# jetuk/pycllp

Hardware: AMD Instinct MI355X
Metric: LPs solved/sec (higher is better)
Workload: dtype f64

## Files before the change

### pycllp_amd/csrc/ipm_group.inc

```

#ifndef PYCLLP_SPLITJ
#define PYCLLP_SPLITJ 6
#endif
#ifndef PYCLLP_GRAM_UNROLL
#define PYCLLP_GRAM_UNROLL 4
#endif
#ifndef PYCLLP_AT_RB
#define PYCLLP_AT_RB 4
#endif
#ifndef PYCLLP_A_CB
#define PYCLLP_A_CB 8
#endif
#ifndef PYCLLP_SOLVE_PRIO
#define PYCLLP_SOLVE_PRIO 2
#endif
#ifndef PYCLLP_FACTOR_PRIO
#define PYCLLP_FACTOR_PRIO 2
#endif
#ifndef PYCLLP_FACTOR_PRIO_HSD
#define PYCLLP_FACTOR_PRIO_HSD 3
#endif
#ifndef PYCLLP_WPB
#define PYCLLP_WPB 8
#endif

template <int MP, int NP, bool SL = false>
struct GeoG {
    static_assert(MP == 16 || MP == 32, "row padding must be 16 or 32");
    static_assert(NP % MP == 0 && NP % 8 == 0 && NP <= 128, "column padding must be a multiple of MP and 8, <= 128");
    static_assert(!SL || NP >= 2 * MP, "the slack-aware variant needs at least one dense register");
    static constexpr int G = 64 / MP;
    static constexpr int NCG = NP / MP;
    static constexpr int ND = SL ? NP - MP : NP;
    static constexpr int NCD = ND / MP;
    static constexpr int JB = MP / 16;
    static constexpr int KS = ND / 4;
    static constexpr int AS = ND + 1;
    static constexpr int AIMG = MP * AS;
    static constexpr bool SWZ = (MP == 32);
    static constexpr int MS = SWZ ? MP : MP + 2;
    __host__ __device__ static constexpr int sidx(int row, int col) {
        return SWZ ? row * MS + (col ^ ((row & 15) << 1)) : row * MS + col;
    }
    static constexpr int SLAB = MP * MS;
    static constexpr int STAGE = 3 * ND;
    static constexpr int STAGE_A = (G * ND > STAGE) ? G * ND : STAGE;
    static constexpr int STAGE_SZ = (2 * G * MP > STAGE_A) ? 2 * G * MP : STAGE_A;
    static constexpr int SHARED = AIMG + ND;
    static constexpr int WSZ = G * SLAB + STAGE_SZ;
    static constexpr size_t lds_bytes(int wpb) { return sizeof(double) * (size_t)(SHARED + wpb * WSZ); }
    __host__ __device__ static constexpr int kpos(int j) { return (j & 3) * KS + (j >> 2); }
};

template <int MP>
__device__ __forceinline__ double grp_sum(double v) {
    asm volatile("" : "+v"(v));
    v += dpp_d<0xB1>(v);
    v += dpp_d<0x4E>(v);
    v += dpp_d<0x141>(v);
    v += dpp_d<0x140>(v);
    if (MP == 32) v += swz_xor16_d(v);
    return v;
}
template <int MP>
__device__ __forceinline__ double grp_max(double v) {
    v = fmax(v, dpp_d<0xB1>(v));
    v = fmax(v, dpp_d<0x4E>(v));
    v = fmax(v, dpp_d<0x141>(v));
    v = fmax(v, dpp_d<0x140>(v));
    if (MP == 32) v = fmax(v, swz_xor16_d(v));
    return v;
}
template <int MP>
__device__ __forceinline__ double grp_bcast(double v, int k, int grp) {
    if (MP == 32) {
        const double a = readlane_d(v, k), b = readlane_d(v, 32 + k);
        return grp ? b : a;
    } else {
        const double a = readlane_d(v, k), b = readlane_d(v, 16 + k), c = readlane_d(v, 32 + k), d = readlane_d(v, 48 + k);
        return (grp & 2) ? ((grp & 1) ? d : c) : ((grp & 1) ? b : a);
    }
}

template <int MP, int NP, bool SL = false>
struct GWave {
    using G_ = GeoG<MP, NP, SL>;
    static constexpr int G = G_::G, NCG = G_::NCG, NCD = G_::NCD, ND = G_::ND, JB = G_::JB, KS = G_::KS, AS = G_::AS, MS = G_::MS;

    const double* Aimg;
    static constexpr bool COLB = MP == 32 && NP <= 96;
    static constexpr bool ROWB = COLB && SL;
    unsigned rb[ROWB ? 16 : 1];
    unsigned xb[COLB ? 16 : 1];
    double* slab;
    double* slab0;
    double* stage;
    int lane, gl, grp, m, n;

    __device__ __forceinline__ int ogl() const { int g = gl; asm volatile("" : "+v"(g)); return g; }

    __device__ __forceinline__ void load_own_row(double (&out)[MP]) const {
        typedef double double2_t __attribute__((ext_vector_type(2)));
        if constexpr (ROWB) {
#pragma unroll
            for (int p2 = 0; p2 < MP / 2; p2++) {
                const double2_t t = *(const __attribute__((address_space(3))) double2_t*)(size_t)rb[p2];
                out[2 * p2] = t[0]; out[2 * p2 + 1] = t[1];
            }
            return;
        }
        const int g = ogl();
        const double2_t* rp = (const double2_t*)(slab + g * MS);
        const int g15 = G_::SWZ ? (g & 15) : 0;
#pragma unroll
        for (int p2 = 0; p2 < MP / 2; p2++) {
            const double2_t t = rp[p2 ^ g15];
            out[2 * p2] = t[0]; out[2 * p2 + 1] = t[1];
        }
    }

    __device__ __forceinline__ void At_times(double u, double (&out)[NCG]) const {
        const int g = ogl();
        stage[grp * MP + g] = u;
        wave_lds_sync();
        unsigned uba = lds_addr(stage + grp * MP);
        asm volatile("" : "+v"(uba));
        const __attribute__((address_space(3))) double* ub = (const __attribute__((address_space(3))) double*)(size_t)uba;
        const double* ac = Aimg + g;
        constexpr int RB = PYCLLP_AT_RB, NB = MP / RB;
        double a0[RB][NCD], a1[RB][NCD], u0[RB], u1[RB];
#define AT_LOAD(A_, U_, I0)                                                                     \
    _Pragma("unroll") for (int ii = 0; ii < RB; ii++) {                                         \
        U_[ii] = ub[(I0) + ii + tok];                                                           \
        _Pragma("unroll") for (int q = 0; q < NCD; q++) A_[ii][q] = ac[((I0) + ii) * AS + MP * q + tok]; \
    }
#define AT_USE(A_, U_)                                                                          \
    _Pragma("unroll") for (int ii = 0; ii < RB; ii++) {                                         \
        asm volatile("" : "+v"(U_[ii]));                                                        \
        _Pragma("unroll") for (int q = 0; q < NCD; q++) asm volatile("" : "+v"(A_[ii][q]));     \
    }                                                                                           \
    asm volatile("" : "+v"(tok));                                                               \
    _Pragma("unroll") for (int ii = 0; ii < RB; ii++)                                           \
        _Pragma("unroll") for (int q = 0; q < NCD; q++) out[q] = fma(A_[ii][q], U_[ii], out[q]); \
    _Pragma("unroll") for (int q = 0; q < NCD; q++) asm volatile("" : "+v"(out[q]));
#pragma unroll
        for (int q = 0; q < NCG; q++) out[q] = 0.0;
        if (SL) out[NCG - 1] = u;
        int tok = 0;
        asm volatile("" : "+v"(tok));
        AT_LOAD(a0, u0, 0)
        static_for<0, NB / 2>([&](auto bc) {
            constexpr int b2 = 2 * decltype(bc)::value;
            AT_LOAD(a1, u1, (b2 + 1) * RB)
            AT_USE(a0, u0)
            if constexpr (b2 + 2 < NB) { AT_LOAD(a0, u0, (b2 + 2) * RB) }
            AT_USE(a1, u1)
        });
#undef AT_LOAD
#undef AT_USE
        wave_lds_sync();
    }

    __device__ __forceinline__ double A_times(const double (&vq)[NCG]) const {
        const int g = ogl();
#pragma unroll
        for (int q = 0; q < NCD; q++) stage[grp * ND + g + MP * q] = vq[q];
        wave_lds_sync();
        unsigned vba = lds_addr(stage + grp * ND);
        asm volatile("" : "+v"(vba));
        const __attribute__((address_space(3))) double* vb = (const __attribute__((address_space(3))) double*)(size_t)vba;
        const double* row = Aimg + g * AS;
        constexpr int CB = (ND % PYCLLP_A_CB == 0) ? PYCLLP_A_CB : 8, NB = ND / CB;
        double a0[CB], a1[CB], v0[CB], v1[CB];
        double acc[4] = {0.0, 0.0, 0.0, 0.0};
#define A_LOAD(A_, V_, J0) \
    _Pragma("unroll") for (int jj = 0; jj < CB; jj++) { A_[jj] = row[(J0) + jj + tok]; V_[jj] = vb[(J0) + jj + tok]; }
#define A_USE(A_, V_)                                                                                          \
    _Pragma("unroll") for (int jj = 0; jj < CB; jj++) { asm volatile("" : "+v"(A_[jj])); asm volatile("" : "+v"(V_[jj])); } \
    asm volatile("" : "+v"(tok));                                                                              \
    _Pragma("unroll") for (int jj = 0; jj < CB; jj++) acc[jj & 3] = fma(A_[jj], V_[jj], acc[jj & 3]);
        int tok = 0;
        asm volatile("" : "+v"(tok));
        A_LOAD(a0, v0, 0)
        static_for<0, (NB + 1) / 2>([&](auto bc) {
            constexpr int b2 = 2 * decltype(bc)::value;
            if constexpr (b2 + 1 < NB) { A_LOAD(a1, v1, (b2 + 1) * CB) }
            A_USE(a0, v0)
            if constexpr (b2 + 2 < NB) { A_LOAD(a0, v0, (b2 + 2) * CB) }
            if constexpr (b2 + 1 < NB) { A_USE(a1, v1) }
        });
#undef A_LOAD
#undef A_USE
        wave_lds_sync();
        return (acc[0] + acc[1]) + (acc[2] + acc[3]) + (SL ? vq[NCG - 1] : 0.0);
    }

    template <bool AX = true>
    __device__ __forceinline__ void gram_one(int g, double (&axp)[JB], double (&adp)[JB]) const {
        int lo0_ = lane;
        asm volatile("" : "+v"(lo0_));
        const int kg = lo0_ >> 4, cc = lo0_ & 15;
        double4_t acc[JB][JB];
#pragma unroll
        for (int I = 0; I < JB; I++) {
            axp[I] = 0.0; adp[I] = 0.0;
#pragma unroll
            for (int J = 0; J < JB; J++) acc[I][J] = (double4_t){0.0, 0.0, 0.0, 0.0};
        }
        const double* px = stage + kg * KS;
        const double* pd = stage + ND + kg * KS;
        const double* pt = stage + 2 * ND + kg * KS;
        const double* arow = Aimg + cc * AS + kg;
        constexpr int SC = (KS % 4 == 0) ? 4 : 2;
#pragma unroll PYCLLP_GRAM_UNROLL
        for (int s0 = 0; s0 < KS; s0 += SC) {
#pragma unroll
            for (int ss = 0; ss < SC; ss++) {
                const int s = s0 + ss;
                const double xk = AX ? px[s] : 0.0, dk = pd[s], tk = pt[s];
                double a[JB], ad[JB];
#pragma unroll
                for (int J = 0; J < JB; J++) {
                    a[J] = arow[16 * J * AS + 4 * s];
                    if (AX) axp[J] = fma(a[J], xk, axp[J]);
                    adp[J] = fma(a[J], tk, adp[J]);
                    ad[J] = a[J] * dk;
                }
#pragma unroll
                for (int I = 0; I < JB; I++)
#pragma unroll
                    for (int J = 0; J <= I; J++)
                        acc[I][J] = __builtin_amdgcn_mfma_f64_16x16x4f64(ad[I], a[J], acc[I][J], 0, 0, 0);
            }
        }
        double* sg = slab0 + g * G_::SLAB;
        int lo_ = lane;
        asm volatile("" : "+v"(lo_));
        const int kg2 = lo_ >> 4, cc2 = lo_ & 15;
        if constexpr (G_::SWZ) {
            const int c0 = cc2 ^ (kg2 << 1);
            double* e0 = sg + kg2 * G_::MS + c0;
            double* e1 = sg + kg2 * G_::MS + (c0 ^ 8);
#pragma unroll
            for (int I = 0; I < JB; I++)
#pragma unroll
                for (int J = 0; J <= I; J++)
#pragma unroll
                    for (int r4 = 0; r4 < 4; r4++)
                        ((r4 & 1) ? e1 : e0)[(16 * I + 4 * r4) * G_::MS + 16 * (J ^ (r4 >> 1))] = acc[I][J][r4];
        } else {
#pragma unroll
            for (int I = 0; I < JB; I++)
#pragma unroll
                for (int J = 0; J <= I; J++)
#pragma unroll
                    for (int r4 = 0; r4 < 4; r4++) {
                        const int row = 16 * I + kg2 + 4 * r4, col = 16 * J + cc2;
                        sg[G_::sidx(row, col)] = acc[I][J][r4];
                    }
        }
#pragma unroll
        for (int J = 0; J < JB; J++) {
            if (AX) {
                axp[J] += __shfl_xor(axp[J], 16, WAVE);
                axp[J] += __shfl_xor(axp[J], 32, WAVE);
            }
            adp[J] += __shfl_xor(adp[J], 16, WAVE);
            adp[J] += __shfl_xor(adp[J], 32, WAVE);
        }
    }

    __device__ __forceinline__ static double top_row_of(double u) {
        const int lo = __double2loint(u), hi = __double2hiint(u);
        auto a = __builtin_amdgcn_permlane16_swap(lo, lo, false, false);
        auto b = __builtin_amdgcn_permlane16_swap(hi, hi, false, false);
        return __hiloint2double(b[0], a[0]);
    }

    template <bool RELF = false>
    __device__ __forceinline__ bool factor_dpp(double (&W)[MP], double beta2, double floor_, bool live, double& rdiag,
                                               const double* fl = nullptr) const {
        rdiag = 1.0;
        constexpr int PRIO_ = RELF ? PYCLLP_FACTOR_PRIO_HSD : PYCLLP_FACTOR_PRIO;
        if constexpr (PRIO_ != 0) __builtin_amdgcn_s_setprio(PRIO_);
        const int go = ogl();
        (void)go;
        double ymax = 0.0;
        static_for<0, MP>([&](auto jc) {
            constexpr int j = decltype(jc)::value;
            const double u = W[j];
            double src = u;
            if constexpr (MP == 32 && j < 16) src = top_row_of(u);
            const double piv = bcast64<j % 16>(src);
            const double aD = RELF ? max_abs<false>(piv, fl[j]) : max_abs<true>(piv, floor_);
            const double rD = fast_rcp(aD);
            constexpr unsigned below32 = (j + 1 < 32) ? (0xFFFFFFFFu << ((j + 1) & 31)) : 0u;
            constexpr unsigned below16 = (j + 1 < 16) ? (((0xFFFFu << ((j + 1) & 15)) & 0xFFFFu) * 0x10001u) : 0u;
            constexpr unsigned MB_ = (MP == 32) ? below32 : below16;
            constexpr unsigned ONE_ = (MP == 32) ? (1u << (j % 32)) : ((1u << (j % 16)) * 0x10001u);
            double l = 0.0;
            asm volatile("" : "+v"(l));
            if constexpr (MP == 16) {
                chain_step_exec<j, MB_, MB_, 1, ONE_, ONE_>(W, 0.0, rD, l, ymax, rdiag);
            } else if constexpr (j < 16) {
                chain_step_exec<j, MB_, MB_, 0, ONE_, ONE_>(*reinterpret_cast<double (*)[16]>(&W[0]), src, rD, l, ymax, rdiag);
                chain_all_neg(*reinterpret_cast<double (*)[16]>(&W[16]), W[j], l);
            } else {
                chain_step_exec<j - 16, MB_, MB_, 1, ONE_, ONE_>(*reinterpret_cast<double (*)[16]>(&W[16]), 0.0, rD, l, ymax, rdiag);
            }
            W[j] = l;
        });
        const bool viol = live && (ymax > beta2);
        if constexpr (PRIO_ != 0) __builtin_amdgcn_s_setprio(0);
        if constexpr (COLB) {
#pragma unroll
            for (int j = 0; j < MP; j++) *(__attribute__((address_space(3))) double*)(size_t)(xb[j & 15] + 256u * (unsigned)(j & ~15)) = W[j];
        } else {
            const int g = ogl();
#pragma unroll
            for (int j = 0; j < MP; j++) slab[G_::sidx(j, g)] = W[j];
        }
        wave_lds_sync();
        return __any(viol);
    }

    __device__ __forceinline__ double factor_guarded_inplace(bool rowok, double beta2, double floor_,
                                                             const double* fl = nullptr) const {
        if (!rowok) slab[G_::sidx(gl, gl)] = 1.0;
        wave_lds_sync();
        double rdiag = 1.0;
#pragma unroll 1
        for (int j = 0; j < MP; j++) {
            const bool below = gl > j;
            const double u = below ? slab[G_::sidx(gl, j)] : 0.0;
            const double piv = slab[G_::sidx(j, j)];
            const double theta = grp_max<MP>(fabs(u));
            const double aD = fmax(fmax(fabs(piv), fl ? fl[j] : floor_), theta * theta / beta2);
            const double rD = fast_rcp(aD);
            const double li = u * rD;
            if (gl == j) rdiag = rD;
#pragma unroll 1
            for (int k = j + 1; k < MP; k++) {
                const double uk = slab[G_::sidx(k, j)];
                if (gl >= k) slab[G_::sidx(gl, k)] = fma(-li, uk, slab[G_::sidx(gl, k)]);
            }
            wave_lds_sync();
            slab[G_::sidx(j, gl)] = below ? li : 0.0;
            wave_lds_sync();
        }
#pragma unroll 1
        for (int k = 0; k < MP; k++) if (k <= gl) slab[G_::sidx(gl, k)] = 0.0;
        wave_lds_sync();
        return rdiag;
    }

    __device__ __forceinline__ double fwd_back(double s, double rdiag) const {
        if constexpr (PYCLLP_SOLVE_PRIO != 0) __builtin_amdgcn_s_setprio(PYCLLP_SOLVE_PRIO);
        double lf[MP];
        if constexpr (COLB) {
#pragma unroll
            for (int k = 0; k < MP - 1; k++) lf[k] = *(const __attribute__((address_space(3))) double*)(size_t)(xb[k & 15] + 256u * (unsigned)(k & ~15));
        } else {
            const int g = ogl();
#pragma unroll
            for (int k = 0; k < MP - 1; k++) lf[k] = slab[G_::sidx(k, g)];
        }
#pragma unroll
        for (int k = 0; k < MP - 1; k++) asm volatile("" : "+v"(lf[k]));
        if constexpr (MP == 16) {
            subst15_up(s, lf);
        } else {
            const bool top = gl < 16;
            if (top) subst15_up(s, lf);
            const double so = swz_xor16_d(s);
            if (!top) {
                s -= dot16_bcast(so, lf);
                subst15_up(s, lf + 16);
            }
        }
        s *= rdiag;
        double lb[MP];
        load_own_row(lb);
#pragma unroll
        for (int i = 1; i < MP; i++) asm volatile("" : "+v"(lb[i]));
        if constexpr (MP == 16) {
            subst15_down(s, lb);
            return s;
        } else {
            const bool top = gl < 16;
            if (!top) subst15_down(s, lb + 16);
            const double so = swz_xor16_d(s);
            if (top) {
                s -= dot16_bcast(so, lb + 16);
                subst15_down(s, lb);
            }
            if constexpr (PYCLLP_SOLVE_PRIO != 0) __builtin_amdgcn_s_setprio(0);
            return s;
        }
    }
};

template <int MP, int NP, bool SL, bool PC = false>
__global__ void __launch_bounds__(PYCLLP_WPB * 64)
ipm_group_kernel(int m, int n, long B, const double* __restrict__ Ag, const double* __restrict__ bg,
                 const double* __restrict__ cg, double* __restrict__ xg, double* __restrict__ yg,
                 double* __restrict__ zg, double* __restrict__ pobj, double* __restrict__ dobj,
                 int* __restrict__ status, int* __restrict__ iters, int* __restrict__ queue, DevOpts o) {
    using G_ = GeoG<MP, NP, SL>;
    constexpr int G = G_::G, NCG = G_::NCG, NCD = G_::NCD, ND = G_::ND, JB = G_::JB, AS = G_::AS;
    const int nd = SL ? n - m : n;
    extern __shared__ __attribute__((aligned(16))) double lds[];
    const int tid = threadIdx.x;
    const int wpb = blockDim.x / WAVE;
    double* Aimg = lds;
    double* colsum = lds + G_::AIMG;
    for (int i = tid; i < G_::AIMG; i += blockDim.x) {
        const int r = i / AS, cidx = i % AS;
        Aimg[i] = (r < m && cidx < nd) ? Ag[(size_t)r * n + cidx] : 0.0;
    }
    __syncthreads();
    for (int j = tid; j < ND; j += blockDim.x) {
        double sacc = 0.0;
        for (int i = 0; i < MP; i++) sacc += Aimg[i * AS + j];
        colsum[j] = sacc;
    }
    __syncthreads();

    GWave<MP, NP, SL> w;
    const int wave = tid / WAVE;
    const int lane = tid & 63, gl = lane & (MP - 1), grp = lane / MP;
    w.lane = lane; w.gl = gl; w.grp = grp; w.m = m; w.n = n;
    w.Aimg = Aimg;
    w.slab0 = lds + G_::SHARED + wave * G_::WSZ;
    w.slab = w.slab0 + grp * G_::SLAB;
    w.stage = w.slab0 + G * G_::SLAB;
    if constexpr (GWave<MP, NP, SL>::COLB) {
#pragma unroll
        for (int cidx = 0; cidx < 16; cidx++) w.xb[cidx] = lds_addr(w.slab) + 8u * (unsigned)G_::sidx(cidx, gl);
    }
    if constexpr (GWave<MP, NP, SL>::ROWB) {
#pragma unroll
        for (int p2 = 0; p2 < 16; p2++) w.rb[p2] = lds_addr(w.slab + gl * G_::MS) + 16u * (unsigned)(p2 ^ (gl & 15));
    }
    for (int i = lane; i < G * G_::SLAB; i += WAVE) w.slab0[i] = 0.0;
    wave_lds_sync();
    const bool rowok = gl < m;
    const bool warm = (o.flags & PYCLLP_FLAG_WARM_START) != 0;
    const bool autoscale = (o.flags & PYCLLP_FLAG_AUTOSCALE) != 0;
    const unsigned long long gmask = (MP == 32) ? 0xFFFFFFFFull : 0xFFFFull;
    STAMP_DECL

    const long nslots = (long)gridDim.x * wpb * G;
    long lp = (long)grp * ((long)gridDim.x * wpb) + (long)blockIdx.x * wpb + wave;
    bool live = lp < B, fresh = live;

    double x[NCG], z[NCG], c[NCG], v[NCG];
    bool ok[NCG];
#pragma unroll
    for (int q = 0; q < NCG; q++) {
        ok[q] = (q < NCD) ? (gl + MP * q < nd) : (gl < m);
        x[q] = 1.0; z[q] = 1.0; c[q] = 0.0; v[q] = 0.0;
    }
    auto gcol = [&](int q, int g_) { return (q < NCD) ? g_ + MP * q : nd + g_; };
    double b = 0.0, y = 0.0;
    double tol_r = 0.0, tol_s = 0.0, etol = 0.0, normr0 = 1e300, norms0 = 1e300;
    double rho_pred = 0.0;
    bool have_pred = false;
    int it = 0;

    while (__any(live)) {
        if (__any(fresh)) {
            if (fresh) {
                const int go = w.ogl();
#pragma unroll
                for (int q = 0; q < NCG; q++) {
                    const int j = gcol(q, go);
                    c[q] = ok[q] ? cg[lp * n + j] : 0.0;
                    x[q] = (warm && ok[q]) ? xg[lp * n + j] : 1.0;
                    z[q] = (warm && ok[q]) ? zg[lp * n + j] : 1.0;
                    v[q] = (q < NCD) ? colsum[go + MP * q] : (rowok ? 1.0 : 0.0);
                }
                b = rowok ? bg[lp * m + go] : 0.0;
                y = rowok ? ((warm && yg) ? yg[lp * m + go] : 1.0) : 0.0;
            }
            if (autoscale) {
                double cm = 0.0;
#pragma unroll
                for (int q = 0; q < NCG; q++) cm = fmax(cm, fabs(c[q]));
                double sb = grp_max<MP>(fabs(b)), sc = grp_max<MP>(cm);
                sb = (sb > 0.0) ? sb : 1.0; sc = (sc > 0.0) ? sc : 1.0;
                if (fresh) {
                    b = b / sb;
#pragma unroll
                    for (int q = 0; q < NCG; q++) c[q] = c[q] / sc;
                    if (warm) {
                        y = y / sc;
#pragma unroll
                        for (int q = 0; q < NCG; q++) { x[q] = x[q] / sb; z[q] = z[q] / sc; }
                    }
                }
            }
            double c2 = 0.0;
#pragma unroll
            for (int q = 0; q < NCG; q++) c2 = fma(c[q], c[q], c2);
            const double nb2 = grp_sum<MP>(b * b), nc2 = grp_sum<MP>(c2);
            double vw[NCG];
            if (warm) w.At_times(y, vw);
            if (fresh) {
                tol_r = o.eps * (1.0 + sqrt(nb2));
                tol_s = o.eps * (1.0 + sqrt(nc2));
                etol = o.refine_tol * (1.0 + sqrt(nb2));
                normr0 = 1e300; norms0 = 1e300; it = 0; have_pred = false;
                if (warm) {
#pragma unroll
                    for (int q = 0; q < NCG; q++) v[q] = vw[q];
                }
            }
            fresh = false;
            STAMP(9)
        }

        double s2 = 0.0, gam = 0.0, pp = 0.0;
#pragma unroll
        for (int q = 0; q < NCG; q++) {
            const double sg = ok[q] ? c[q] - v[q] + z[q] : 0.0;
            s2 = fma(sg, sg, s2);
            gam += ok[q] ? x[q] * z[q] : 0.0;
            pp += c[q] * (ok[q] ? x[q] : 0.0);
        }
        s2 = grp_sum<MP>(s2); gam = grp_sum<MP>(gam);
        const double po = grp_sum<MP>(pp);
        const double du = grp_sum<MP>(b * y);
        const double norms = sqrt(s2);
        double mu = PC ? 0.0 : o.delta * gam / (double)(n + m);

        auto finalize = [&](int stat_) {
            double sb = 1.0, sc = 1.0;
            const int go = w.ogl();
            int gro = grp;
            asm volatile("" : "+v"(gro));
            if (autoscale) {
                double cm = 0.0;
#pragma unroll
                for (int q = 0; q < NCG; q++) cm = fmax(cm, ok[q] ? fabs(cg[lp * n + gcol(q, go)]) : 0.0);
                sb = grp_max<MP>(rowok ? fabs(bg[lp * m + go]) : 0.0);
                sc = grp_max<MP>(cm);
                sb = (sb > 0.0) ? sb : 1.0; sc = (sc > 0.0) ? sc : 1.0;
            }
#pragma unroll
            for (int q = 0; q < NCG; q++) {
                const int j = gcol(q, go);
                if (ok[q]) {
                    xg[lp * n + j] = x[q] * sb;
                    if (zg) zg[lp * n + j] = z[q] * sc;
                }
            }
            if (yg && rowok) yg[lp * m + go] = y * sc;
            if (go == 0) {
                if (pobj) pobj[lp] = po * (sb * sc);
                if (dobj) dobj[lp] = du * (sb * sc);
                status[lp] = stat_;
                if (iters) iters[lp] = it;
            }
            int nxt = 0;
            if (go == 0) nxt = atomicAdd(queue, 1);
            nxt = __shfl(nxt, gro * MP, WAVE);
            lp = nslots + (long)nxt;
            live = lp < B;
            fresh = live;
            have_pred = false;
            if (!live) {
#pragma unroll
// ... 215 lines not shown
```

### pycllp_amd/csrc/ipm_group_bounded.inc

```

#ifndef PYCLLP_WPB_BOUNDED
#define PYCLLP_WPB_BOUNDED 4
#endif

template <int MP, int NP>
__global__ void __launch_bounds__(PYCLLP_WPB_BOUNDED * 64)
ipm_bounded_kernel(int m, int n, long B, const double* __restrict__ Ag, const double* __restrict__ bg,
                   const double* __restrict__ cg, const double* __restrict__ ug, double* __restrict__ xg,
                   double* __restrict__ yg, double* __restrict__ zg, double* __restrict__ sg, double* __restrict__ pobj,
                   double* __restrict__ dobj, int* __restrict__ status, int* __restrict__ iters, int* __restrict__ queue,
                   DevOpts o) {
    using G_ = GeoG<MP, NP, true>;
    constexpr int G = G_::G, NCG = G_::NCG, NCD = G_::NCD, ND = G_::ND, JB = G_::JB, AS = G_::AS;
    const int nd = n - m;
    extern __shared__ __attribute__((aligned(16))) double lds[];
    const int tid = threadIdx.x;
    const int wpb = blockDim.x / WAVE;
    double* Aimg = lds;
    double* colsum = lds + G_::AIMG;
    for (int i = tid; i < G_::AIMG; i += blockDim.x) {
        const int r = i / AS, cidx = i % AS;
        Aimg[i] = (r < m && cidx < nd) ? Ag[(size_t)r * n + cidx] : 0.0;
    }
    __syncthreads();
    for (int j = tid; j < ND; j += blockDim.x) {
        double sacc = 0.0;
        for (int i = 0; i < MP; i++) sacc += Aimg[i * AS + j];
        colsum[j] = sacc;
    }
    __syncthreads();

    GWave<MP, NP, true> w;
    const int wave = tid / WAVE;
    const int lane = tid & 63, gl = lane & (MP - 1), grp = lane / MP;
    w.lane = lane; w.gl = gl; w.grp = grp; w.m = m; w.n = n;
    w.Aimg = Aimg;
    w.slab0 = lds + G_::SHARED + wave * G_::WSZ;
    w.slab = w.slab0 + grp * G_::SLAB;
    w.stage = w.slab0 + G * G_::SLAB;
    if constexpr (GWave<MP, NP, true>::COLB) {
#pragma unroll
        for (int cidx = 0; cidx < 16; cidx++) w.xb[cidx] = lds_addr(w.slab) + 8u * (unsigned)G_::sidx(cidx, gl);
    }
    if constexpr (GWave<MP, NP, true>::ROWB) {
#pragma unroll
        for (int p2 = 0; p2 < 16; p2++) w.rb[p2] = lds_addr(w.slab + gl * G_::MS) + 16u * (unsigned)(p2 ^ (gl & 15));
    }
    for (int i = lane; i < G * G_::SLAB; i += WAVE) w.slab0[i] = 0.0;
    wave_lds_sync();
    const bool rowok = gl < m;
    const bool autoscale = (o.flags & PYCLLP_FLAG_AUTOSCALE) != 0;
    const unsigned long long gmask = (MP == 32) ? 0xFFFFFFFFull : 0xFFFFull;

    const long nslots = (long)gridDim.x * wpb * G;
    long lp = (long)grp * ((long)gridDim.x * wpb) + (long)blockIdx.x * wpb + wave;
    bool live = lp < B, fresh = live;

    double x[NCG], z[NCG], t[NCG], s[NCG], u[NCG], c[NCG], v[NCG];
    bool ok[NCG];
#pragma unroll
    for (int q = 0; q < NCG; q++) {
        ok[q] = (q < NCD) ? (gl + MP * q < nd) : (gl < m);
        x[q] = 1.0; z[q] = 1.0; t[q] = 1.0; s[q] = 1.0; u[q] = 0.0; c[q] = 0.0; v[q] = 0.0;
    }
    auto act = [&](int q) { return u[q] > 0.0; };
    auto bnd = [&](int q) { return u[q] > 0.0 && u[q] < HUGE_VAL; };
    auto gcol = [&](int q, int g_) { return (q < NCD) ? g_ + MP * q : nd + g_; };
    double b = 0.0, y = 0.0;
    double tol_r = 0.0, tol_s = 0.0, tol_u = 0.0, etol = 0.0, normr0 = 1e300, norms0 = 1e300, ncomp = 1.0;
    int it = 0;

    while (__any(live)) {
        if (__any(fresh)) {
            if (fresh) {
                const int go = w.ogl();
#pragma unroll
                for (int q = 0; q < NCG; q++) {
                    const int j = gcol(q, go);
                    c[q] = ok[q] ? cg[lp * n + j] : 0.0;
                    u[q] = ok[q] ? ug[lp * n + j] : 0.0;
                    v[q] = (q < NCD) ? colsum[go + MP * q] : (rowok ? 1.0 : 0.0);
                }
                b = rowok ? bg[lp * m + go] : 0.0;
                y = rowok ? 1.0 : 0.0;
            }
            if (autoscale) {
                double cm = 0.0;
#pragma unroll
                for (int q = 0; q < NCG; q++) cm = fmax(cm, act(q) ? fabs(c[q]) : 0.0);
                double sb = grp_max<MP>(fabs(b)), sc = grp_max<MP>(cm);
                sb = (sb > 0.0) ? sb : 1.0; sc = (sc > 0.0) ? sc : 1.0;
                if (fresh) {
                    b = b / sb;
#pragma unroll
                    for (int q = 0; q < NCG; q++) { c[q] = c[q] / sc; u[q] = u[q] / sb; }
                }
            }
            double c2 = 0.0, u2 = 0.0, nb = 0.0;
#pragma unroll
            for (int q = 0; q < NCG; q++) {
                c2 += act(q) ? c[q] * c[q] : 0.0;
                u2 += bnd(q) ? u[q] * u[q] : 0.0;
                nb += bnd(q) ? 1.0 : 0.0;
            }
            const double nb2 = grp_sum<MP>(b * b), nc2 = grp_sum<MP>(c2), nu2 = grp_sum<MP>(u2), nbs = grp_sum<MP>(nb);
            if (fresh) {
#pragma unroll
                for (int q = 0; q < NCG; q++) {
                    x[q] = bnd(q) ? fmin(1.0, 0.5 * u[q]) : 1.0;
                    t[q] = bnd(q) ? u[q] - x[q] : 1.0;
                    z[q] = 1.0; s[q] = 1.0;
                }
                tol_r = o.eps * (1.0 + sqrt(nb2));
                tol_s = o.eps * (1.0 + sqrt(nc2));
                tol_u = o.eps * (1.0 + sqrt(nu2));
                etol = o.refine_tol * (1.0 + sqrt(nb2));
                ncomp = (double)(n + m) + nbs;
                normr0 = 1e300; norms0 = 1e300; it = 0;
            }
            fresh = false;
        }

        double s2 = 0.0, gam = 0.0, pp = 0.0, tau2 = 0.0, du = b * y;
#pragma unroll
        for (int q = 0; q < NCG; q++) {
            const bool a = act(q), bq = bnd(q);
            const double sgq = a ? c[q] - v[q] + z[q] - (bq ? s[q] : 0.0) : 0.0;
            const double tau = bq ? (u[q] - x[q]) - t[q] : 0.0;
            s2 = fma(sgq, sgq, s2);
            tau2 = fma(tau, tau, tau2);
            gam += a ? x[q] * z[q] : 0.0;
            gam += bq ? s[q] * t[q] : 0.0;
            pp += a ? c[q] * x[q] : 0.0;
            du += bq ? u[q] * s[q] : 0.0;
        }
        s2 = grp_sum<MP>(s2); gam = grp_sum<MP>(gam); tau2 = grp_sum<MP>(tau2);
        const double po = grp_sum<MP>(pp);
        du = grp_sum<MP>(du);
        const double norms = sqrt(s2), ntau = sqrt(tau2);
        const double mu = o.delta * gam / ncomp;

        auto finalize = [&](int stat_) {
            double sb = 1.0, sc = 1.0;
            const int go = w.ogl();
            int gro = grp;
            asm volatile("" : "+v"(gro));
            if (autoscale) {
                double cm = 0.0;
#pragma unroll
                for (int q = 0; q < NCG; q++) cm = fmax(cm, act(q) ? fabs(cg[lp * n + gcol(q, go)]) : 0.0);
                sb = grp_max<MP>(rowok ? fabs(bg[lp * m + go]) : 0.0);
                sc = grp_max<MP>(cm);
                sb = (sb > 0.0) ? sb : 1.0; sc = (sc > 0.0) ? sc : 1.0;
            }
#pragma unroll
            for (int q = 0; q < NCG; q++) {
                const int j = gcol(q, go);
                if (ok[q]) {
                    const bool a = act(q), bq = bnd(q);
                    const double r = c[q] - v[q];
                    xg[lp * n + j] = a ? x[q] * sb : 0.0;
                    if (zg) zg[lp * n + j] = (a ? z[q] : fmax(-r, 0.0)) * sc;
                    if (sg) sg[lp * n + j] = (bq ? s[q] : (a ? 0.0 : fmax(r, 0.0))) * sc;
                }
            }
            if (yg && rowok) yg[lp * m + go] = y * sc;
            if (go == 0) {
                if (pobj) pobj[lp] = po * (sb * sc);
                if (dobj) dobj[lp] = du * (sb * sc);
                status[lp] = stat_;
                if (iters) iters[lp] = it;
            }
            int nxt = 0;
            if (go == 0) nxt = atomicAdd(queue, 1);
            nxt = __shfl(nxt, gro * MP, WAVE);
            lp = nslots + (long)nxt;
            live = lp < B;
            fresh = live;
            if (!live) {
#pragma unroll
                for (int q = 0; q < NCG; q++) { x[q] = 1.0; z[q] = 1.0; t[q] = 1.0; s[q] = 1.0; u[q] = 0.0; c[q] = 0.0; v[q] = 0.0; }
                b = 0.0; y = 0.0;
            }
        };

        double rxk[NCG], rzk[NCG], rtk[NCG];
#pragma unroll
        for (int q = 0; q < NCG; q++) { rxk[q] = fast_rcp(x[q]); rzk[q] = fast_rcp(z[q]); rtk[q] = fast_rcp(t[q]); }
        auto newton_dt = [&](int q, double& dq, double& tq) {
            const bool a = act(q), bq = bnd(q);
            const double tau = (u[q] - x[q]) - t[q];
            if (bq) {
                dq = fast_rcp(fma(z[q], rxk[q], s[q] * rtk[q]));
                tq = c[q] - v[q] + mu * rxk[q] - mu * rtk[q] + (s[q] * rtk[q]) * tau;
            } else {
                dq = x[q] * rzk[q];
                tq = c[q] - v[q] + mu * rxk[q];
            }
            dq = a ? dq : 0.0;
            tq = a ? tq : 0.0;
        };
        auto do_gram = [&](double& Ax_, double& Adt_) {
            double d[NCG], tt[NCG];
#pragma unroll
            for (int q = 0; q < NCG; q++) newton_dt(q, d[q], tt[q]);
#pragma unroll 1
            for (int g = 0; g < G; g++) {
                if (__shfl((int)live, g * MP, WAVE) == 0) continue;
                if (grp == g) {
#pragma unroll
                    for (int q = 0; q < NCD; q++) {
                        const int p = G_::kpos(gl + MP * q);
                        w.stage[p] = act(q) ? x[q] : 0.0;
                        w.stage[ND + p] = d[q];
                        w.stage[2 * ND + p] = d[q] * tt[q];
                    }
                }
                wave_lds_sync();
                double axp[JB], adp[JB];
                w.template gram_one<true>(g, axp, adp);
                wave_lds_sync();
                if (grp == g) {
                    Ax_ = (JB == 1) ? axp[0] : ((gl >> 4) ? axp[JB - 1] : axp[0]);
                    Adt_ = (JB == 1) ? adp[0] : ((gl >> 4) ? adp[JB - 1] : adp[0]);
                }
            }
            Ax_ += act(NCG - 1) ? x[NCG - 1] : 0.0;
            Adt_ += d[NCG - 1] * tt[NCG - 1];
            w.slab[G_::sidx(gl, gl)] += d[NCG - 1];
            wave_lds_sync();
        };
        double Ax = 0.0, Adt = 0.0;
        do_gram(Ax, Adt);
        const double rho = b - Ax;
        const double normr = sqrt(grp_sum<MP>(rho * rho));

        int stat = PYCLLP_STATUS_ITERATION_LIMIT;
        bool fin = true;
        if (!(isfinite(normr) && isfinite(norms) && isfinite(gam) && isfinite(ntau))) stat = PYCLLP_STATUS_NUMERICAL;
        else if (normr <= tol_r && norms <= tol_s && gam <= o.eps * (1.0 + fabs(po)) && ntau <= tol_u) stat = PYCLLP_STATUS_OPTIMAL;
        else if (normr > 10.0 * normr0 && normr > PYCLLP_GROWTH_FLOOR * tol_r) stat = PYCLLP_STATUS_PRIMAL_INFEASIBLE;
        else if (norms > 10.0 * norms0 && norms > PYCLLP_GROWTH_FLOOR * tol_s) stat = PYCLLP_STATUS_DUAL_INFEASIBLE;
        else fin = false;
        const bool work = live && !fin;

        const double rhs = Adt - rho;
        double rdiag;
        {
            double W[MP];
            const int gd = w.ogl();
            if (m < MP) {
                if (!rowok) w.slab[G_::sidx(gd, gd)] = 1.0;
                wave_lds_sync();
            }
            w.load_own_row(W);
            double diag = rowok ? w.slab[G_::sidx(gd, gd)] : 0.0;
            const double beta2 = grp_max<MP>(fabs(diag));
            wave_lds_sync();
            const bool redo = w.factor_dpp(W, beta2, o.pivot_floor, work, rdiag);
            if (redo || (o.flags & PYCLLP_FLAG_FORCE_GUARD_PATH)) {
                double Ax2, Adt2;
                do_gram(Ax2, Adt2);
                rdiag = w.factor_guarded_inplace(rowok, beta2, o.pivot_floor);
            }
        }
        double dy = w.fwd_back(rhs, rdiag);
        double wv[NCG], dx[NCG], d[NCG];
        w.At_times(dy, wv);
#pragma unroll
        for (int q = 0; q < NCG; q++) {
            double tq;
            newton_dt(q, d[q], tq);
            dx[q] = (tq - wv[q]) * d[q];
        }
        int nref = 0;
        for (;;) {
            const double e = rho - w.A_times(dx);
            const double maxe = grp_max<MP>(fabs(e));
            const bool need = work && (maxe > etol) && (nref < o.max_refine);
            if (!__any(need)) break;
            const double eta = w.fwd_back(need ? e : 0.0, rdiag);
            double w2[NCG];
            w.At_times(eta, w2);
#pragma unroll
            for (int q = 0; q < NCG; q++) {
                dx[q] = fma(d[q], w2[q], dx[q]);
                wv[q] -= w2[q];
            }
            dy -= eta;
            nref += need ? 1 : 0;
        }
        const unsigned long long nf = __ballot(!isfinite(dy));
        const bool dy_bad = ((nf >> (grp * MP)) & gmask) != 0ull;
        if (!fin && dy_bad) { fin = true; stat = PYCLLP_STATUS_NUMERICAL; }

        if (!fin) {
            double dz[NCG], dt[NCG], ds[NCG];
            double th = 0.0;
#pragma unroll
            for (int q = 0; q < NCG; q++) {
                const bool a = act(q), bq = bnd(q);
                const double tau = (u[q] - x[q]) - t[q];
                dz[q] = a ? (mu - z[q] * dx[q]) * rxk[q] - z[q] : 0.0;
                dt[q] = bq ? tau - dx[q] : 0.0;
                ds[q] = bq ? (mu - s[q] * dt[q]) * rtk[q] - s[q] : 0.0;
                if (a) th = fmax(th, fmax(-dz[q] * rzk[q], -dx[q] * rxk[q]));
                if (bq) th = fmax(th, fmax(-dt[q] * rtk[q], -ds[q] * fast_rcp(s[q])));
            }
            th = grp_max<MP>(th);
            const double theta = fmin(o.r / th, 1.0);
            y = fma(theta, dy, y);
#pragma unroll
            for (int q = 0; q < NCG; q++) {
                const bool a = act(q), bq = bnd(q);
                x[q] = a ? fma(theta, dx[q], x[q]) : x[q];
                z[q] = a ? fma(theta, dz[q], z[q]) : z[q];
                t[q] = bq ? fma(theta, dt[q], t[q]) : t[q];
                s[q] = bq ? fma(theta, ds[q], s[q]) : s[q];
                v[q] = fma(theta, wv[q], v[q]);
            }
            normr0 = normr; norms0 = norms;
            it++;
            if (it >= o.max_iter) fin = true;
        }
        if (fin && live) finalize(stat);
    }
}
```

### pycllp_amd/csrc/ipm_group_hsd.inc

```

#ifndef PYCLLP_HSD_AT_RB
#define PYCLLP_HSD_AT_RB 4
#endif
template <int MP, int NP, bool SL>
struct GWaveH : GWave<MP, NP, SL> {
    using Base = GWave<MP, NP, SL>;
    using G_ = GeoG<MP, NP, SL>;
    static constexpr int G = G_::G, NCG = G_::NCG, NCD = G_::NCD, AS = G_::AS, MS = G_::MS;

    __device__ __forceinline__ void At_times2(double u1, double u2, double (&o1)[NCG], double (&o2)[NCG]) const {
        const int g = this->ogl();
        this->stage[this->grp * MP + g] = u1;
        this->stage[G * MP + this->grp * MP + g] = u2;
        wave_lds_sync();
        unsigned uba = lds_addr(this->stage + this->grp * MP);
        asm volatile("" : "+v"(uba));
        const __attribute__((address_space(3))) double* ub = (const __attribute__((address_space(3))) double*)(size_t)uba;
        const double* ac = this->Aimg + g;
        constexpr int RB = PYCLLP_HSD_AT_RB, NB = MP / RB;
        double a0[RB][NCD], a1[RB][NCD], u0[RB][2], u1_[RB][2];
#define AT_LOAD(A_, U_, I0)                                                                     \
    _Pragma("unroll") for (int ii = 0; ii < RB; ii++) {                                         \
        U_[ii][0] = ub[(I0) + ii + tok];                                                        \
        U_[ii][1] = ub[G * MP + (I0) + ii + tok];                                               \
        _Pragma("unroll") for (int q = 0; q < NCD; q++) A_[ii][q] = ac[((I0) + ii) * AS + MP * q + tok]; \
    }
#define AT_USE(A_, U_)                                                                          \
    _Pragma("unroll") for (int ii = 0; ii < RB; ii++) {                                         \
        asm volatile("" : "+v"(U_[ii][0]));                                                     \
        asm volatile("" : "+v"(U_[ii][1]));                                                     \
        _Pragma("unroll") for (int q = 0; q < NCD; q++) asm volatile("" : "+v"(A_[ii][q]));     \
    }                                                                                           \
    asm volatile("" : "+v"(tok));                                                               \
    _Pragma("unroll") for (int ii = 0; ii < RB; ii++)                                           \
        _Pragma("unroll") for (int q = 0; q < NCD; q++) {                                       \
            o1[q] = fma(A_[ii][q], U_[ii][0], o1[q]);                                           \
            o2[q] = fma(A_[ii][q], U_[ii][1], o2[q]);                                           \
        }                                                                                       \
     \
     \
    _Pragma("unroll") for (int q = 0; q < NCD; q++) { asm volatile("" : "+v"(o1[q])); asm volatile("" : "+v"(o2[q])); }
#pragma unroll
        for (int q = 0; q < NCG; q++) { o1[q] = 0.0; o2[q] = 0.0; }
        if (SL) { o1[NCG - 1] = u1; o2[NCG - 1] = u2; }
        int tok = 0;
        asm volatile("" : "+v"(tok));
        AT_LOAD(a0, u0, 0)
        static_for<0, NB / 2>([&](auto bc) {
            constexpr int b2 = 2 * decltype(bc)::value;
            AT_LOAD(a1, u1_, (b2 + 1) * RB)
            AT_USE(a0, u0)
            if constexpr (b2 + 2 < NB) { AT_LOAD(a0, u0, (b2 + 2) * RB) }
            AT_USE(a1, u1_)
        });
#undef AT_LOAD
#undef AT_USE
        wave_lds_sync();
    }

    __device__ __forceinline__ void fwd_back2(double& s, double& t, double rdiag) const {
        const int gl = this->gl;
        const int g = this->ogl();
        const double* slab = this->slab;
        double lf[MP];
        if constexpr (Base::COLB) {
#pragma unroll
            for (int k = 0; k < MP - 1; k++) lf[k] = *(const __attribute__((address_space(3))) double*)(size_t)(this->xb[k & 15] + 256u * (unsigned)(k & ~15));
        } else {
#pragma unroll
            for (int k = 0; k < MP - 1; k++) lf[k] = slab[G_::sidx(k, g)];
        }
#pragma unroll
        for (int k = 0; k < MP - 1; k++) asm volatile("" : "+v"(lf[k]));
        if constexpr (MP == 16) {
            subst15_up2(s, t, lf);
        } else {
            const bool top = gl < 16;
            if (top) subst15_up2(s, t, lf);
            const double so = swz_xor16_d(s), to = swz_xor16_d(t);
            if (!top) {
                s -= dot16_bcast(so, lf); t -= dot16_bcast(to, lf);
                subst15_up2(s, t, lf + 16);
            }
        }
        s *= rdiag; t *= rdiag;
        double lb[MP];
        this->load_own_row(lb);
#pragma unroll
        for (int i = 1; i < MP; i++) asm volatile("" : "+v"(lb[i]));
        if constexpr (MP == 16) {
            subst15_down2(s, t, lb);
        } else {
            const bool top = gl < 16;
            if (!top) subst15_down2(s, t, lb + 16);
            const double so = swz_xor16_d(s), to = swz_xor16_d(t);
            if (top) {
                s -= dot16_bcast(so, lb + 16); t -= dot16_bcast(to, lb + 16);
                subst15_down2(s, t, lb);
            }
        }
    }
};

#ifndef PYCLLP_WPB_HSD
#define PYCLLP_WPB_HSD 8
#endif
template <int MP> constexpr int hsd_wpb() { return MP == 16 ? PYCLLP_WPB : PYCLLP_WPB_HSD; }

template <int MP, int NP, bool SL>
__global__ void __launch_bounds__(hsd_wpb<MP>() * 64)
hsd_group_kernel(int m, int n, long B, const double* __restrict__ Ag, const double* __restrict__ bg,
                 const double* __restrict__ cg, double* __restrict__ xg, double* __restrict__ yg,
                 double* __restrict__ zg, double* __restrict__ pobj, double* __restrict__ dobj,
                 int* __restrict__ status, int* __restrict__ iters, int* __restrict__ queue, DevOpts o) {
    using G_ = GeoG<MP, NP, SL>;
    constexpr int G = G_::G, NCG = G_::NCG, NCD = G_::NCD, ND = G_::ND, JB = G_::JB, AS = G_::AS;
    const int nd = SL ? n - m : n;
    extern __shared__ __attribute__((aligned(16))) double lds[];
    const int tid = threadIdx.x;
    const int wpb = blockDim.x / WAVE;
    double* Aimg = lds;
    for (int i = tid; i < G_::AIMG; i += blockDim.x) {
        const int r = i / AS, cidx = i % AS;
        Aimg[i] = (r < m && cidx < nd) ? Ag[(size_t)r * n + cidx] : 0.0;
    }
    __syncthreads();

    GWaveH<MP, NP, SL> w;
    const int wave = __builtin_amdgcn_readfirstlane(tid / WAVE);
    const int lane = tid & 63, gl = lane & (MP - 1), grp = lane / MP;
    w.lane = lane; w.gl = gl; w.grp = grp; w.m = m; w.n = n;
    w.Aimg = Aimg;
    w.slab0 = lds + G_::SHARED + wave * G_::WSZ;
    w.slab = w.slab0 + grp * G_::SLAB;
    w.stage = w.slab0 + G * G_::SLAB;
    if constexpr (GWave<MP, NP, SL>::COLB) {
#pragma unroll
        for (int cidx = 0; cidx < 16; cidx++) w.xb[cidx] = lds_addr(w.slab) + 8u * (unsigned)G_::sidx(cidx, gl);
    }
    if constexpr (GWave<MP, NP, SL>::ROWB) {
#pragma unroll
        for (int p2 = 0; p2 < 16; p2++) w.rb[p2] = lds_addr(w.slab + gl * G_::MS) + 16u * (unsigned)(p2 ^ (gl & 15));
    }
    for (int i = lane; i < G * G_::SLAB; i += WAVE) w.slab0[i] = 0.0;
    wave_lds_sync();
    const bool rowok = gl < m;
    const bool warm = (o.flags & PYCLLP_FLAG_WARM_START) != 0;
    const bool autoscale = (o.flags & PYCLLP_FLAG_AUTOSCALE) != 0;
    const unsigned long long gmask = (MP == 32) ? 0xFFFFFFFFull : 0xFFFFull;
#define HSD_ETA (1.0 - sopaque(o.delta))
#define HSD_EINF (100.0 * sopaque(o.eps))

    const long nslots = (long)gridDim.x * wpb * G;
    long lp = (long)grp * ((long)gridDim.x * wpb) + (long)blockIdx.x * wpb + wave;
    bool live = lp < B, fresh = live;

    double x[NCG], z[NCG], c[NCG], v[NCG];
    bool ok[NCG];
#pragma unroll
    for (int q = 0; q < NCG; q++) {
        ok[q] = (q < NCD) ? (gl + MP * q < nd) : (gl < m);
        x[q] = 1.0; z[q] = 1.0; c[q] = 0.0; v[q] = 0.0;
    }
    auto gcol = [&](int q, int g_) { return (q < NCD) ? g_ + MP * q : nd + g_; };
    double b = 0.0, y = 0.0, tau = 1.0, kap = 1.0, nb = 0.0, nc = 0.0;
    int it = 0;

    while (__any(live)) {
        if (__any(fresh)) {
            if (fresh) {
                const int go = w.ogl();
#pragma unroll
                for (int q = 0; q < NCG; q++) {
                    const int j = gcol(q, go);
                    c[q] = ok[q] ? cg[lp * n + j] : 0.0;
                    x[q] = (warm && ok[q]) ? xg[lp * n + j] : 1.0;
                    z[q] = (warm && ok[q]) ? zg[lp * n + j] : 1.0;
                    v[q] = 0.0;
                }
                b = rowok ? bg[lp * m + go] : 0.0;
                y = (rowok && warm && yg) ? yg[lp * m + go] : 0.0;
            }
            if (autoscale) {
                double cm = 0.0;
#pragma unroll
                for (int q = 0; q < NCG; q++) cm = fmax(cm, fabs(c[q]));
                double sb = grp_max<MP>(fabs(b)), sc = grp_max<MP>(cm);
                sb = (sb > 0.0) ? sb : 1.0; sc = (sc > 0.0) ? sc : 1.0;
                if (fresh) {
                    b = b / sb;
#pragma unroll
                    for (int q = 0; q < NCG; q++) c[q] = c[q] / sc;
                    if (warm) {
                        y = y / sc;
#pragma unroll
                        for (int q = 0; q < NCG; q++) { x[q] = x[q] / sb; z[q] = z[q] / sc; }
                    }
                }
            }
            double c2 = 0.0, g0 = 0.0;
#pragma unroll
            for (int q = 0; q < NCG; q++) {
                c2 = fma(c[q], c[q], c2);
                g0 += ok[q] ? x[q] * z[q] : 0.0;
            }
            const double nb2 = grp_sum<MP>(b * b), nc2 = grp_sum<MP>(c2);
            g0 = grp_sum<MP>(g0);
            double vw[NCG];
            if (warm) w.At_times(y, vw);
            if (fresh) {
                nb = sqrt(nb2); nc = sqrt(nc2);
                tau = 1.0;
                kap = warm ? g0 / (double)n : 1.0;
                it = 0;
                if (warm) {
#pragma unroll
                    for (int q = 0; q < NCG; q++) v[q] = vw[q];
                }
            }
            fresh = false;
        }

        double rho;
        {
            double xm[NCG];
#pragma unroll
            for (int q = 0; q < NCG; q++) xm[q] = ok[q] ? x[q] : 0.0;
            rho = fma(b, tau, -w.A_times(xm));
        }
        double s2 = 0.0, gam = 0.0, pp = 0.0;
#pragma unroll
        for (int q = 0; q < NCG; q++) {
            const double sg = ok[q] ? fma(c[q], tau, z[q] - v[q]) : 0.0;
            s2 = fma(sg, sg, s2);
            gam += ok[q] ? x[q] * z[q] : 0.0;
            pp += c[q] * (ok[q] ? x[q] : 0.0);
        }
        s2 = grp_sum<MP>(s2); gam = grp_sum<MP>(gam);
        const double po = grp_sum<MP>(pp);
        const double du = grp_sum<MP>(b * y);
        const double norms = sqrt(s2);
        const double normr = sqrt(grp_sum<MP>(rho * rho));

        auto finalize = [&](int stat_) {
            double sb = 1.0, sc = 1.0;
            const int go = w.ogl();
            int gro = grp;
            asm volatile("" : "+v"(gro));
            if (autoscale) {
                double cm = 0.0;
#pragma unroll
                for (int q = 0; q < NCG; q++) cm = fmax(cm, ok[q] ? fabs(cg[lp * n + gcol(q, go)]) : 0.0);
                sb = grp_max<MP>(rowok ? fabs(bg[lp * m + go]) : 0.0);
                sc = grp_max<MP>(cm);
                sb = (sb > 0.0) ? sb : 1.0; sc = (sc > 0.0) ? sc : 1.0;
            }
            const double rt = (stat_ == PYCLLP_STATUS_OPTIMAL || stat_ == PYCLLP_STATUS_ITERATION_LIMIT) ? 1.0 / tau : 1.0;
#pragma unroll
            for (int q = 0; q < NCG; q++) {
                const int j = gcol(q, go);
                if (ok[q]) {
                    xg[lp * n + j] = x[q] * rt * sb;
                    if (zg) zg[lp * n + j] = z[q] * rt * sc;
                }
            }
            if (yg && rowok) yg[lp * m + go] = y * rt * sc;
            if (go == 0) {
                if (pobj) pobj[lp] = po * rt * (sb * sc);
                if (dobj) dobj[lp] = du * rt * (sb * sc);
                status[lp] = stat_;
                if (iters) iters[lp] = it;
            }
            int nxt = 0;
            if (go == 0) nxt = atomicAdd(queue, 1);
            nxt = __shfl(nxt, gro * MP, WAVE);
            lp = nslots + (long)nxt;
            live = lp < B;
            fresh = live;
// ... 185 lines not shown
```

Baseline: 11.64 million.

## Compute diagonal Gram blocks with 4x4 MFMAs and an LDS scatter table

For MP=32, the three 16x16x4 f64 MFMAs that covered the two diagonal 16x16 blocks (including wasted upper-triangle work) are replaced by one 16x16 MFMA for the off-diagonal block plus five 4x4x4 MFMAs. These five cover exactly the lower-triangular 4x4 tiles of the diagonal blocks. A per-block LDS table of scatter offsets is filled at kernel start so each lane can store its 4x4 results into the swizzled slab. The intent is to cut redundant MFMA throughput in the Gram product, at the cost of extra LDS reads (wrapped A rows, the offset table) and some added LDS footprint. The MP=16 path is reduced to a single accumulator.

```diff
diff --git a/pycllp_amd/csrc/ipm_group.inc b/pycllp_amd/csrc/ipm_group.inc
--- a/pycllp_amd/csrc/ipm_group.inc
+++ b/pycllp_amd/csrc/ipm_group.inc
@@ -24,6 +24,26 @@
 #define PYCLLP_WPB 8
 #endif
 
+struct GramPair { int own, par; };
+constexpr int GRAM_INSTS = 5;
+constexpr GramPair gram_pair(int r, int b) {
+    return r == 0 ? GramPair{b, b} : r == 1 ? GramPair{b + 4, b + 4} : r == 2 ? GramPair{b, (b + 3) & 3}
+         : r == 3 ? GramPair{b + 4, 4 + ((b + 3) & 3)} : (b < 2 ? GramPair{b, b + 2} : GramPair{b + 4, b + 2});
+}
+constexpr bool gram_pairs_cover_diagonal_blocks() {
+    int cnt[8][8] = {};
+    for (int r = 0; r < GRAM_INSTS; r++)
+        for (int b = 0; b < 4; b++) {
+            const GramPair t = gram_pair(r, b);
+            cnt[t.own > t.par ? t.own : t.par][t.own > t.par ? t.par : t.own]++;
+        }
+    for (int i = 0; i < 8; i++)
+        for (int j = 0; j < 8; j++)
+            if (cnt[i][j] != ((j <= i && i / 4 == j / 4) ? 1 : 0)) return false;
+    return true;
+}
+static_assert(gram_pairs_cover_diagonal_blocks(), "the five instructions must cover the 20 lower tiles of the diagonal blocks exactly once");
+
 template <int MP, int NP, bool SL = false>
 struct GeoG {
     static_assert(MP == 16 || MP == 32, "row padding must be 16 or 32");
@@ -46,7 +66,23 @@
     static constexpr int STAGE = 3 * ND;
     static constexpr int STAGE_A = (G * ND > STAGE) ? G * ND : STAGE;
     static constexpr int STAGE_SZ = (2 * G * MP > STAGE_A) ? 2 * G * MP : STAGE_A;
-    static constexpr int SHARED = AIMG + ND;
+    __host__ __device__ static constexpr int gram_store(int r, int lane) {
+        const GramPair t = gram_pair(r, (lane >> 2) & 3);
+        const int ro = 4 * t.own + (lane >> 4), rp = 4 * t.par + (lane & 3);
+        return 8 * (t.par > t.own ? sidx(rp, ro) : sidx(ro, rp));
+    }
+    __host__ __device__ static constexpr int gram_wrap(int lane) { return 8 * AS * (((lane & 15) + 12) & 15); }
+    static constexpr int GROWS = GRAM_INSTS + 1;
+    static constexpr int GTAB = (MP == 32) ? GROWS * 64 / 4 : 0;
+    static constexpr int GTAB_OFF = AIMG + ND;
+    __device__ static void fill_gram_table(double* lds, int tid, int nthreads) {
+        if constexpr (MP == 32) {
+            unsigned short* tab = (unsigned short*)(lds + GTAB_OFF);
+            for (int i = tid; i < GROWS * 64; i += nthreads)
+                tab[i] = (unsigned short)(i < GRAM_INSTS * 64 ? gram_store(i >> 6, i & 63) : gram_wrap(i & 63));
+        }
+    }
+    static constexpr int SHARED = GTAB_OFF + GTAB;
     static constexpr int WSZ = G * SLAB + STAGE_SZ;
     static constexpr size_t lds_bytes(int wpb) { return sizeof(double) * (size_t)(SHARED + wpb * WSZ); }
     __host__ __device__ static constexpr int kpos(int j) { return (j & 3) * KS + (j >> 2); }
@@ -195,69 +231,90 @@
         return (acc[0] + acc[1]) + (acc[2] + acc[3]) + (SL ? vq[NCG - 1] : 0.0);
     }
 
-    template <bool AX = true>
+    template <bool AX = true, bool LATE = false>
     __device__ __forceinline__ void gram_one(int g, double (&axp)[JB], double (&adp)[JB]) const {
         int lo0_ = lane;
         asm volatile("" : "+v"(lo0_));
         const int kg = lo0_ >> 4, cc = lo0_ & 15;
-        double4_t acc[JB][JB];
-#pragma unroll
-        for (int I = 0; I < JB; I++) {
-            axp[I] = 0.0; adp[I] = 0.0;
-#pragma unroll
-            for (int J = 0; J < JB; J++) acc[I][J] = (double4_t){0.0, 0.0, 0.0, 0.0};
-        }
+#pragma unroll
+        for (int I = 0; I < JB; I++) { axp[I] = 0.0; adp[I] = 0.0; }
         const double* px = stage + kg * KS;
         const double* pd = stage + ND + kg * KS;
         const double* pt = stage + 2 * ND + kg * KS;
         const double* arow = Aimg + cc * AS + kg;
+        double* sg = slab0 + g * G_::SLAB;
         constexpr int SC = (KS % 4 == 0) ? 4 : 2;
+        if constexpr (MP == 32) {
+            const unsigned short* tab = (const unsigned short*)(Aimg + G_::GTAB_OFF) + lo0_;
+            const __attribute__((address_space(3))) double* wrow =
+                (const __attribute__((address_space(3))) double*)(size_t)(lds_addr(Aimg + kg) + tab[64 * GRAM_INSTS]);
+            unsigned so[GRAM_INSTS];
+            if constexpr (!LATE) {
+#pragma unroll
+                for (int r = 0; r < GRAM_INSTS; r++) so[r] = tab[64 * r];
+            }
+            const bool top = cc < 8;
+            double4_t acc10 = (double4_t){0.0, 0.0, 0.0, 0.0};
+            double acc[GRAM_INSTS];
+#pragma unroll
+            for (int r = 0; r < GRAM_INSTS; r++) acc[r] = 0.0;
 #pragma unroll PYCLLP_GRAM_UNROLL
-        for (int s0 = 0; s0 < KS; s0 += SC) {
-#pragma unroll
-            for (int ss = 0; ss < SC; ss++) {
-                const int s = s0 + ss;
-                const double xk = AX ? px[s] : 0.0, dk = pd[s], tk = pt[s];
-                double a[JB], ad[JB];
-#pragma unroll
-                for (int J = 0; J < JB; J++) {
-                    a[J] = arow[16 * J * AS + 4 * s];
-                    if (AX) axp[J] = fma(a[J], xk, axp[J]);
-                    adp[J] = fma(a[J], tk, adp[J]);
-                    ad[J] = a[J] * dk;
-                }
-#pragma unroll
-                for (int I = 0; I < JB; I++)
-#pragma unroll
-                    for (int J = 0; J <= I; J++)
-                        acc[I][J] = __builtin_amdgcn_mfma_f64_16x16x4f64(ad[I], a[J], acc[I][J], 0, 0, 0);
-            }
-        }
-        double* sg = slab0 + g * G_::SLAB;
-        int lo_ = lane;
-        asm volatile("" : "+v"(lo_));
-        const int kg2 = lo_ >> 4, cc2 = lo_ & 15;
-        if constexpr (G_::SWZ) {
-            const int c0 = cc2 ^ (kg2 << 1);
+            for (int s0 = 0; s0 < KS; s0 += SC) {
+#pragma unroll
+                for (int ss = 0; ss < SC; ss++) {
+                    const int s = s0 + ss;
+                    const double xk = AX ? px[s] : 0.0, dk = pd[s], tk = pt[s];
+                    double a[2], ad[2];
+#pragma unroll
+                    for (int J = 0; J < 2; J++) {
+                        a[J] = arow[16 * J * AS + 4 * s];
+                        if (AX) axp[J] = fma(a[J], xk, axp[J]);
+                        adp[J] = fma(a[J], tk, adp[J]);
+                        ad[J] = a[J] * dk;
+                    }
+                    const double p3 = wrow[4 * s], p7 = wrow[16 * AS + 4 * s], p2 = arow[8 * AS + 4 * s];
+                    acc10 = __builtin_amdgcn_mfma_f64_16x16x4f64(ad[1], a[0], acc10, 0, 0, 0);
+                    acc[0] = __builtin_amdgcn_mfma_f64_4x4x4f64(ad[0], a[0], acc[0], 0, 0, 0);
+                    acc[1] = __builtin_amdgcn_mfma_f64_4x4x4f64(ad[1], a[1], acc[1], 0, 0, 0);
+                    acc[2] = __builtin_amdgcn_mfma_f64_4x4x4f64(ad[0], p3, acc[2], 0, 0, 0);
+                    acc[3] = __builtin_amdgcn_mfma_f64_4x4x4f64(ad[1], p7, acc[3], 0, 0, 0);
+                    acc[4] = __builtin_amdgcn_mfma_f64_4x4x4f64(top ? ad[0] : ad[1], p2, acc[4], 0, 0, 0);
+                }
+            }
+            int lo_ = lane;
+            asm volatile("" : "+v"(lo_));
+            if constexpr (LATE) {
+                const unsigned short* tab2 = (const unsigned short*)(Aimg + G_::GTAB_OFF) + lo_;
+#pragma unroll
+                for (int r = 0; r < GRAM_INSTS; r++) so[r] = tab2[64 * r];
+            }
+            const unsigned sga = lds_addr(sg);
+#pragma unroll
+            for (int r = 0; r < GRAM_INSTS; r++) *(__attribute__((address_space(3))) double*)(size_t)(sga + so[r]) = acc[r];
+            const int kg2 = lo_ >> 4, c0 = (lo_ & 15) ^ (kg2 << 1);
             double* e0 = sg + kg2 * G_::MS + c0;
             double* e1 = sg + kg2 * G_::MS + (c0 ^ 8);
 #pragma unroll
-            for (int I = 0; I < JB; I++)
-#pragma unroll
-                for (int J = 0; J <= I; J++)
-#pragma unroll
-                    for (int r4 = 0; r4 < 4; r4++)
-                        ((r4 & 1) ? e1 : e0)[(16 * I + 4 * r4) * G_::MS + 16 * (J ^ (r4 >> 1))] = acc[I][J][r4];
+            for (int r4 = 0; r4 < 4; r4++) ((r4 & 1) ? e1 : e0)[(16 + 4 * r4) * G_::MS + 16 * (r4 >> 1)] = acc10[r4];
         } else {
-#pragma unroll
-            for (int I = 0; I < JB; I++)
-#pragma unroll
-                for (int J = 0; J <= I; J++)
-#pragma unroll
-                    for (int r4 = 0; r4 < 4; r4++) {
-                        const int row = 16 * I + kg2 + 4 * r4, col = 16 * J + cc2;
-                        sg[G_::sidx(row, col)] = acc[I][J][r4];
-                    }
+            double4_t acc = (double4_t){0.0, 0.0, 0.0, 0.0};
+#pragma unroll PYCLLP_GRAM_UNROLL
+            for (int s0 = 0; s0 < KS; s0 += SC) {
+#pragma unroll
+                for (int ss = 0; ss < SC; ss++) {
+                    const int s = s0 + ss;
+                    const double xk = AX ? px[s] : 0.0, dk = pd[s], tk = pt[s];
+                    const double a = arow[4 * s];
+                    if (AX) axp[0] = fma(a, xk, axp[0]);
+                    adp[0] = fma(a, tk, adp[0]);
+                    acc = __builtin_amdgcn_mfma_f64_16x16x4f64(a * dk, a, acc, 0, 0, 0);
+                }
+            }
+            int lo_ = lane;
+            asm volatile("" : "+v"(lo_));
+            const int kg2 = lo_ >> 4, cc2 = lo_ & 15;
+#pragma unroll
+            for (int r4 = 0; r4 < 4; r4++) sg[G_::sidx(kg2 + 4 * r4, cc2)] = acc[r4];
         }
 #pragma unroll
         for (int J = 0; J < JB; J++) {
@@ -418,6 +475,7 @@
         const int r = i / AS, cidx = i % AS;
         Aimg[i] = (r < m && cidx < nd) ? Ag[(size_t)r * n + cidx] : 0.0;
     }
+    G_::fill_gram_table(lds, tid, blockDim.x);
     __syncthreads();
     for (int j = tid; j < ND; j += blockDim.x) {
         double sacc = 0.0;
diff --git a/pycllp_amd/csrc/ipm_group_bounded.inc b/pycllp_amd/csrc/ipm_group_bounded.inc
--- a/pycllp_amd/csrc/ipm_group_bounded.inc
+++ b/pycllp_amd/csrc/ipm_group_bounded.inc
@@ -22,6 +22,7 @@
         const int r = i / AS, cidx = i % AS;
         Aimg[i] = (r < m && cidx < nd) ? Ag[(size_t)r * n + cidx] : 0.0;
     }
+    G_::fill_gram_table(lds, tid, blockDim.x);
     __syncthreads();
     for (int j = tid; j < ND; j += blockDim.x) {
         double sacc = 0.0;
@@ -218,7 +219,7 @@
                 }
                 wave_lds_sync();
                 double axp[JB], adp[JB];
-                w.template gram_one<true>(g, axp, adp);
+                w.template gram_one<true, true>(g, axp, adp);
                 wave_lds_sync();
                 if (grp == g) {
                     Ax_ = (JB == 1) ? axp[0] : ((gl >> 4) ? axp[JB - 1] : axp[0]);
diff --git a/pycllp_amd/csrc/ipm_group_hsd.inc b/pycllp_amd/csrc/ipm_group_hsd.inc
--- a/pycllp_amd/csrc/ipm_group_hsd.inc
+++ b/pycllp_amd/csrc/ipm_group_hsd.inc
@@ -124,6 +124,7 @@
         const int r = i / AS, cidx = i % AS;
         Aimg[i] = (r < m && cidx < nd) ? Ag[(size_t)r * n + cidx] : 0.0;
     }
+    G_::fill_gram_table(lds, tid, blockDim.x);
     __syncthreads();
 
     GWaveH<MP, NP, SL> w;
```

Result: faster. 11.95 million, median of 6 (+2.6%).
